# cliarie/radix-join

Hardware: AMD Instinct MI355X
Metric: probe_tuples_per_sec (higher is better)
Workload: dtype int32

## Files before the change

radix-join_amd/csrc/rj_context.hip:

```cpp
#include <dlfcn.h>

#include <algorithm>
#include <chrono>
#include <cstdlib>

#include "rj_internal.hpp"

namespace rj {

[[noreturn]] void launch_failed(const char* kernel, const char* what, bool unsupported) {
    throw_fmt(unsupported ? RJ_ERR_UNSUPPORTED : RJ_ERR_DEVICE, "launch %s: %s", kernel, what);
}

static int env_int(const char* name, int def) {
    const char* v = getenv(name);
    return v && *v ? atoi(v) : def;
}

void Tuning::from_env() {
    blocked_mid = env_int("RJ_TUNE_BLOCKED_MID", blocked_mid);
    mall_chunk = env_int("RJ_TUNE_MALL_CHUNK", mall_chunk);
    radix_bits = env_int("RJ_TUNE_RADIX_BITS", radix_bits);
    p1_bits = env_int("RJ_TUNE_P1_BITS", p1_bits);
    fine = env_int("RJ_TUNE_FINE", fine);
    pack = env_int("RJ_TUNE_PACK", pack);
    aos3 = env_int("RJ_TUNE_AOS3", aos3);
    aos_mid = env_int("RJ_TUNE_AOS_MID", aos_mid);
    tpg1 = env_int("RJ_TUNE_TPG1", tpg1);
    xcd_split = env_int("RJ_TUNE_XCD_SPLIT", xcd_split);
    tpg2 = env_int("RJ_TUNE_TPG2", tpg2);
    packed_side = env_int("RJ_TUNE_PACKED_SIDE", packed_side);
    xcd_min_rows = env_int("RJ_TUNE_XCD_MIN_ROWS", xcd_min_rows);
    spec_p1 = env_int("RJ_TUNE_SPEC_P1", spec_p1);
    spec_min_rows = env_int("RJ_TUNE_SPEC_MIN_ROWS", spec_min_rows);
    spec_sample = std::min(5, std::max(1, env_int("RJ_TUNE_SPEC_SAMPLE", spec_sample)));
    spec_z = std::max(0, env_int("RJ_TUNE_SPEC_Z", spec_z));
    spec_p2 = env_int("RJ_TUNE_SPEC_P2", spec_p2);
    spec2_min_rows = env_int("RJ_TUNE_SPEC2_MIN_ROWS", spec2_min_rows);
    spec2_sample = std::min(4, std::max(1, env_int("RJ_TUNE_SPEC2_SAMPLE", spec2_sample)));
    spec2_z = std::max(0, env_int("RJ_TUNE_SPEC2_Z", spec2_z));
    bcast = env_int("RJ_TUNE_BCAST", bcast);
    diag = env_int("RJ_DIAG", diag);
    varchar_dev_rows = env_int("RJ_TUNE_VARCHAR_DEV", varchar_dev_rows);
    vkey_hash_bits = env_int("RJ_DEBUG_VKEY_HASH_BITS", vkey_hash_bits);
    sync_upload = env_int("RJ_SYNC_UPLOAD", sync_upload);
    wide_carry = env_int("RJ_TUNE_WIDE_CARRY", wide_carry);
    fold_owner = env_int("RJ_TUNE_FOLD_OWNER", fold_owner);
    group_grid = env_int("RJ_TUNE_GROUP_GRID", group_grid);
    win_grid = env_int("RJ_TUNE_WIN_GRID", win_grid);
    map_grid = env_int("RJ_TUNE_MAP_GRID", map_grid);
    setop_grid = env_int("RJ_TUNE_SETOP_GRID", setop_grid);
    exchange_timeout_ms = env_int("RJ_EXCHANGE_TIMEOUT_MS", exchange_timeout_ms);
    bringup_timeout_ms = env_int("RJ_BRINGUP_TIMEOUT_MS", bringup_timeout_ms);
    debug_shard_fail = env_int("RJ_DEBUG_SHARD_FAIL", debug_shard_fail);
    debug_shard_fail_rank = env_int("RJ_DEBUG_SHARD_FAIL_RANK", debug_shard_fail_rank);
    if (const char* v = getenv("RJ_DEBUG_POISON"))
        debug_poison = (int)strtol(v, nullptr, 0) & 0x1ff;
}

static size_t round_size(size_t n) {
    const size_t small = 256, big = size_t(2) << 20;
    if (n < (size_t(1) << 20)) return (n + small - 1) / small * small;
    return (n + big - 1) / big * big;
}

void* DevPool::alloc(size_t bytes) {
    size_t need = round_size(bytes ? bytes : 1);
    int    best = -1;
    for (size_t i = 0; i < blocks_.size(); ++i) {
        Block& b = blocks_[i];
        if (!b.free || b.size < need) continue;
        if (b.size > need + need / 2 + (size_t(4) << 20)) continue;
        if (best < 0 || b.size < blocks_[best].size) best = (int)i;
    }
    if (best >= 0) {
        if (poison_) {
            hipError_t e = fill(blocks_[best].p, blocks_[best].size);
            if (e != hipSuccess) throw_fmt(RJ_ERR_DEVICE, "RJ_DEBUG_POISON: fill on alloc failed: %s", hipGetErrorString(e));
        }
        blocks_[best].free = false;
        in_use_ += blocks_[best].size;
        cached_ -= blocks_[best].size;
        return blocks_[best].p;
    }
    void*      p = nullptr;
    auto       t0 = std::chrono::steady_clock::now();
    hipError_t e = hipMalloc(&p, need);
    if (e != hipSuccess) {
        (void)hipGetLastError();
// ... 265 lines not shown
```

radix-join_amd/csrc/rj_internal.hpp:

```cpp
#pragma once
#include <hip/hip_runtime.h>

#include <atomic>
#include <cstdarg>
#include <cstdio>
#include <cstring>
#include <functional>
#include <map>
#include <memory>
#include <mutex>
#include <stdexcept>
#include <string>
#include <vector>

#include "../../include/rj.h"
#include "rj_comm.hpp"
#include "rj_device.hpp"
#include "rj_kernels.hpp"

namespace rj {

struct Context;

struct Error : std::runtime_error {
// ... 111 lines not shown
    uint64_t       page_rows_total = 0;
    BufP           page_rows;
    std::vector<uint32_t> page_rows_host;
    std::vector<uint8_t>        host_pages;
    std::vector<const uint8_t*> vc_pages;
    mutable BufP vc_dev, vc_dev_dir;
    bool                        skipped = false;
};

struct Table {
    Context*                 ctx = nullptr;
    uint64_t                 num_rows = 0;
    std::vector<TableColumn> cols;
};

struct ResultColumn {
    int32_t              type = 0;
    uint64_t             n_pages = 0;
    BufP                 dev_pages;
    std::vector<uint8_t> host_pages;
    struct Part {
        Context* ctx;
        BufP     pages;
        uint64_t n_pages;
    };
    std::vector<Part> more;
    uint64_t          n_first = 0;
};

struct Result {
    Context*                  ctx = nullptr;
    uint64_t                  num_rows = 0;
    std::vector<ResultColumn> cols;
};

struct Tuning {
    int blocked_mid = 1;
    int mall_chunk = 0;
    int radix_bits = 0;
    int p1_bits = 0;
    int fine = 1;
    int pack = 1;
    int aos3 = 1;
    int aos_mid = 2;
    int tpg1 = 0;
    int packed_side = 0;
    int tpg2 = 0;
    int xcd_min_rows = 40 << 20;
    int xcd_split = 1;
    int spec_p1 = 1;
    int spec_min_rows = 40 << 20;
    int spec_sample = 5;
    int spec_z = 60;
    int spec_p2 = 1;
    int spec2_min_rows = 40 << 20;
    int spec2_sample = 2;
    int spec2_z = 70;
    int bcast = 1;
    int diag = 0;
    int varchar_dev_rows = 200000;
    int vkey_hash_bits = 0;
    int sync_upload = 0;
    int wide_carry = 1;
    int fold_owner = 1;
    int group_grid = 0;
    int map_grid = 0;
    int win_grid = 0;
    int setop_grid = 0;
    int exchange_timeout_ms = 120000;
    int bringup_timeout_ms = 0;
    int debug_shard_fail = 0, debug_shard_fail_rank = 0;
    int debug_poison = 0;
    void from_env();
};

struct Context {
    Tuning      tune;
    int         device = 0;
    hipStream_t stream = nullptr;
    bool        own_stream = false;
    int         radix_bits_override = 0;
    DevPool     pool;
    Profiler    prof;
    LaunchLog   klog;
    std::string last_error;
    void*  pinned = nullptr;
    size_t pinned_bytes = 0;
    static constexpr size_t SMALL_PINNED = 32768;
    void*  pinned_small = nullptr;
    void*  small_pinned();
    hipStream_t copy_stream = nullptr;
    void*       pinned_up = nullptr;
    size_t      pinned_up_bytes = 0;
    hipStream_t upload_stream();
    hipStream_t aux = nullptr;
    hipStream_t aux_stream();
    void*       upload_staging(size_t bytes);
    Launch launch() {
        Launch L;
        L.stream = stream;
        L.self = this;
        L.timed = prof.on ? [](void* s, const char* n, hipEvent_t* a, hipEvent_t* b) {
            return static_cast<Context*>(s)->prof.timed(n, a, b);
        } : (bool (*)(void*, const char*, hipEvent_t*, hipEvent_t*)) nullptr;
        L.logged = klog.on ? [](void* s, const void* k) { static_cast<Context*>(s)->klog.add(k); }
                           : (void (*)(void*, const void*)) nullptr;
// ... 95 lines not shown
```

radix-join_amd/csrc/rj_kernels.hpp:

```cpp
#pragma once
#include <hip/hip_runtime.h>

#include "rj_device.hpp"

namespace rj {

struct Launch {
    hipStream_t stream;
    bool (*timed)(void* self, const char* name, hipEvent_t* start, hipEvent_t* stop);
    void* self;
    void (*logged)(void* self, const void* kernel);
};

[[noreturn]] void launch_failed(const char* kernel, const char* what, bool unsupported);

void launch_page_headers(const Launch& L, const uint8_t* pages, uint32_t n_pages, uint32_t rows_full,
                         uint32_t* page_rows, unsigned long long* flags);
void launch_rows_beyond(const Launch& L, const uint8_t* pages, uint32_t n_pages,
                        const uint32_t* row_base, uint64_t num_rows, unsigned long long* flag);
void launch_decode_pages(const Launch& L, const uint8_t* pages, uint32_t n_pages, int width,
                         const uint32_t* row_base, uint64_t num_rows, uint8_t* values,
                         uint8_t* valid);

void launch_gather(const Launch& L, const ColRef& src, const uint32_t* idx, uint64_t n,
                   const OutStream& dst, uint8_t* dst_valid);
void launch_outer_gather(const Launch& L, const ColRef& src, const uint32_t* idx, uint64_t n, uint8_t* dst,
                         uint8_t* dst_valid);
void launch_finish_pages(const Launch& L, uint8_t* pages, uint64_t n_rows, int width);
void launch_finish_streams(const Launch& L, uint8_t* const* pages, const int* widths, uint32_t n,
                           const unsigned long long* n_rows_dev, uint64_t cap_rows);
void launch_encode_nullable(const Launch& L, const uint8_t* values, const uint8_t* valid,
                            uint64_t n_rows, int width, uint8_t* pages);
void launch_pack_validity(const Launch& L, const uint8_t* v0, const uint8_t* v1, const uint8_t* v2, uint32_t n,
                          uint32_t* out);
void launch_split_records(const Launch& L, const SplitParams& sp, uint64_t n);
void launch_debug_stall(const Launch& L, uint32_t ms);

void launch_scan_bins(const Launch& L, const uint32_t* in, uint32_t n, uint32_t* off,
                      uint32_t* cursor);
void launch_scan_segments(const Launch& L, const uint32_t* hist, const uint32_t* seg_off,
                          uint32_t nseg, uint32_t F, uint32_t xcd_log2, uint32_t* off, uint32_t* cursor);
void launch_group_table(const Launch& L, const uint32_t* seg_off, uint32_t nseg,
                        uint32_t group_tuples, uint32_t* grp_start, const uint32_t* seg_end = nullptr);

void launch_pass_hist_src(const Launch& L, const TupleSrc& src, int key_words, const PassParams& pp,
                          uint32_t n_groups);
void launch_fine_hist_src(const Launch& L, const TupleSrc& src, int key_words, uint32_t shift,
                          uint32_t b1, uint32_t b2, uint32_t grid, uint32_t* fine, uint32_t xcd_tpg = 0,
                          uint32_t* coarse_x = nullptr);
void launch_fine_hist_words(const Launch& L, const Words& in, bool packed, uint32_t n, uint32_t shift,
                            uint32_t b1, uint32_t b2, uint32_t grid, uint32_t* fine, uint32_t xcd_tpg = 0,
                            uint32_t* coarse_x = nullptr);
void launch_scan_fine(const Launch& L, const uint32_t* fine, uint32_t F1, uint32_t F2,
                      uint32_t* off2, uint32_t* cursor2, uint32_t* off1, uint32_t* cursor1,
                      const uint32_t* coarse_x = nullptr);
void launch_pass_scatter_src(const Launch& L, const TupleSrc& src, int key_words, int carry_words,
                             const PassParams& pp, uint32_t n_groups, const Words& out, bool aos3 = false,
                             const SpecParams* spec = nullptr);
void launch_pass_sample_src(const Launch& L, const TupleSrc& src, int key_words, const PassParams& pp,
                            const SpecParams& sp, uint32_t n_groups);
void launch_spec_caps(const Launch& L, const uint32_t* sample, uint32_t nbins, uint32_t sample_log2, float z,
                      uint32_t cap_max, uint32_t* start, uint32_t* limit, unsigned long long* cursor);
void launch_spec_close(const Launch& L, const unsigned long long* cursor, const uint32_t* start, const uint32_t* limit,
                       uint32_t F, uint32_t* seg_end, uint32_t* oseg_off);
void launch_pass_hist_dense(const Launch& L, const Words& in, const PassParams& pp,
                            uint32_t n_groups);
void launch_pass_scatter_dense(const Launch& L, const Words& in, int n_words, int pair_word,
                               const PassParams& pp, uint32_t n_groups, const Words& out, bool aos3 = false);

void launch_pass_hist_digits(const Launch& L, const uint16_t* digits, const PassParams& pp, uint32_t n_groups);
void launch_pass_hist_aos3(const Launch& L, const uint32_t* in_tuples, const PassParams& pp, uint32_t n_groups);
void launch_pass_scatter_aos3(const Launch& L, const uint32_t* in_tuples, const PassParams& pp, uint32_t n_groups,
                              uint32_t* out_tuples);

void launch_pass_hist_packed(const Launch& L, const uint32_t* in_pairs, const PassParams& pp,
                             uint32_t n_groups);
void launch_pass_scatter_src_packed(const Launch& L, const TupleSrc& src, const PassParams& pp,
                                    uint32_t n_groups, uint32_t* out_pairs, bool blocked_out = false,
                                    const SpecParams* spec = nullptr);
void launch_pass_hist_blocked(const Launch& L, const uint32_t* in_blocked, const PassParams& pp, uint32_t n_groups);
void launch_pass_scatter_blocked(const Launch& L, const uint32_t* in_blocked, const PassParams& pp, uint32_t n_groups,
                                 uint32_t* out_pairs, bool blocked_out);
void launch_pass_scatter_packed(const Launch& L, const uint32_t* in_pairs, const PassParams& pp,
                                uint32_t n_groups, uint32_t* out_pairs);

void launch_heavy_tasks(const Launch& L, const uint32_t* offR, const uint32_t* offS, uint32_t NP,
                        uint32_t* tasks, uint32_t* n_heavy, uint32_t max_tasks, uint32_t off_pairs = 0);

void launch_last_sample(const Launch& L, const uint32_t* in_keys, bool blocked, const PassParams& pp, const LastParams& sp,
                        uint32_t n_groups);
void launch_last_caps(const Launch& L, const uint32_t* sample, uint32_t nseg, uint32_t F, uint32_t sample_log2, float z,
                      uint32_t cap_max, unsigned long long* seg_sum, uint32_t* pairs, uint32_t* limit,
                      uint32_t* cursor);
void launch_last_scatter_dense(const Launch& L, const Words& in, const PassParams& pp, uint32_t n_groups, const Words& out,
                               const LastParams& sp);
void launch_last_scatter_blocked(const Launch& L, const uint32_t* in_blocked, const PassParams& pp, uint32_t n_groups,
                                 uint32_t* out_pairs, const LastParams& sp);
void launch_last_close(const Launch& L, const uint32_t* cursor, const uint32_t* limit, uint32_t nbins,
                       uint32_t* pairs);

uint32_t join_partitions_per_workgroup(int key_words, int cw_build, const JoinParams& jp);
void launch_join(const Launch& L, int key_words, int cw_build, int cw_probe, const JoinParams& jp,
                 uint32_t grid);

void launch_join_bcast(const Launch& L, int key_words, int cw_build, int cw_probe,
                       const BcastParams& bp, uint32_t grid);

void launch_filter_bcast(const Launch& L, int key_words, int cw_preserved, const FilterParams& fp, uint32_t grid);
void launch_filter_join(const Launch& L, int key_words, int cw_preserved, const FilterParams& fp, uint32_t grid);
void launch_filter_nullkeys(const Launch& L, int key_words, int cw_preserved, const FilterParams& fp, uint32_t grid);

void launch_outer_bcast(const Launch& L, int key_words, int cw_optional, int cw_preserved, const OuterParams& op,
                        uint32_t grid);
// ... 105 lines not shown
```

radix-join_amd/csrc/rj_pages.hip:

```cpp
#include <hip/hip_ext.h>

#include "rj_kernels.hpp"
#include "rj_kernel_util.hpp"
#include "rj_tuple_util.hpp"

#include <algorithm>
#include <type_traits>

namespace rj {

__global__ __launch_bounds__(256) void k_page_headers(const uint8_t* pages, uint32_t n_pages,
                                                      uint32_t rows_full, uint32_t* page_rows,
                                                      unsigned long long* flags) {
    __shared__ unsigned long long s_irr[4], s_rows[4];
    const uint32_t     lane = threadIdx.x & 63u, wid = threadIdx.x >> 6;
    unsigned long long irr = 0, rows = 0;
    for (uint32_t p = blockIdx.x * 4u + wid; p < n_pages; p += gridDim.x * 4u) {
        const uint8_t* page = pages + (size_t)p * PAGE_BYTES;
        const uint32_t nr = *reinterpret_cast<const uint16_t*>(page);
        const uint32_t nb = (nr + 7) / 8;
        const uint8_t* bm = page + PAGE_BYTES - nb;
        bool           ones = true;
        const uint32_t boff = PAGE_BYTES - nb;
        if ((nr & 31u) == 0 && (boff & 3u) == 0) {
// ... 93 lines not shown
}

template <int WIDTH>
__global__ __launch_bounds__(256) void k_gather(ColRef src, const uint32_t* idx, uint64_t n,
                                                OutStream dst, uint8_t* dst_valid) {
    uint64_t i = (uint64_t)blockIdx.x * blockDim.x + threadIdx.x;
    if (i >= n) return;
    uint32_t r = idx ? idx[i] : (uint32_t)i;
    if (WIDTH == 4) {
        stream_store(dst, i, col_load32(src, r), 0u);
    } else {
        uint64_t v = col_load64(src, r);
        stream_store(dst, i, (uint32_t)v, (uint32_t)(v >> 32));
    }
    if (dst_valid) dst_valid[i] = src.valid ? src.valid[r] : (uint8_t)1;
}

template <int WIDTH>
__global__ __launch_bounds__(256) void k_outer_gather(ColRef src, const uint32_t* idx, uint64_t n, uint8_t* dst,
                                                      uint8_t* dst_valid) {
    const uint64_t i = (uint64_t)blockIdx.x * blockDim.x + threadIdx.x;
    if (i >= n) return;
    const uint32_t r = idx[i];
    const bool     there = r != OUTER_NO_ROW;
    if (WIDTH == 4)
        reinterpret_cast<uint32_t*>(dst)[i] = there ? col_load32(src, r) : 0u;
    else
        reinterpret_cast<uint64_t*>(dst)[i] = there ? col_load64(src, r) : 0ull;
    dst_valid[i] = there ? (src.valid ? src.valid[r] : (uint8_t)1) : (uint8_t)0;
}

__global__ __launch_bounds__(256) void k_finish_pages(uint8_t* pages, uint64_t n_rows,
                                                      uint32_t rows_full) {
    uint8_t*       page = pages + (size_t)blockIdx.x * PAGE_BYTES;
    const uint64_t first = (uint64_t)blockIdx.x * rows_full;
    const uint32_t nr = (uint32_t)min((uint64_t)rows_full, n_rows - first);
    const uint32_t nb = (nr + 7) / 8;
    if (threadIdx.x == 0) {
        reinterpret_cast<uint16_t*>(page)[0] = (uint16_t)nr;
        reinterpret_cast<uint16_t*>(page)[1] = (uint16_t)nr;
    }
    uint8_t* bm = page + PAGE_BYTES - nb;
    for (uint32_t k = threadIdx.x; k < nb; k += blockDim.x) {
        uint32_t bits = nr - k * 8u;
        bm[k] = bits >= 8 ? 0xff : (uint8_t)((1u << bits) - 1u);
    }
}

struct FinishStreams {
    uint8_t* pages[3];
    uint32_t rows_full[3];
    uint32_t n;
};
__global__ __launch_bounds__(256) void k_finish_streams(FinishStreams fs,
                                                        const unsigned long long* n_rows_dev,
                                                        uint64_t cap_rows) {
    const uint64_t n_rows = *n_rows_dev;
    if (n_rows > cap_rows) return;
    const uint32_t b = blockIdx.y, lane = threadIdx.x & 63u;
    const uint32_t rf = fs.rows_full[b];
    const uint64_t pg = (uint64_t)blockIdx.x * (blockDim.x >> 6) + (threadIdx.x >> 6);
    const uint64_t first = pg * rf;
    if (first >= n_rows) return;
    uint8_t*       page = fs.pages[b] + (size_t)pg * PAGE_BYTES;
    const uint32_t nr = (uint32_t)min((uint64_t)rf, n_rows - first);
    const uint32_t nb = (nr + 7) / 8;
    if (lane == 0) *reinterpret_cast<uint32_t*>(page) = nr | (nr << 16);
    uint8_t* bm = page + PAGE_BYTES - nb;
    if (nr == rf && (nr & 31u) == 0 && ((PAGE_BYTES - nb) & 3u) == 0) {
        for (uint32_t k = lane; k < nb / 4; k += 64) reinterpret_cast<uint32_t*>(bm)[k] = 0xffffffffu;
        return;
    }
    if (nr == rf && rf == ROWS64) {
        static_assert(ROWS64 == 1007 && ((PAGE_BYTES - 126 + 2) & 3u) == 0, "bitmap layout of a full 8-byte page");
        if (lane == 0) *reinterpret_cast<uint16_t*>(bm) = 0xffffu;
        if (lane < 31) reinterpret_cast<uint32_t*>(bm + 2)[lane] = lane == 30 ? 0x7fffffffu : 0xffffffffu;
        return;
    }
    for (uint32_t k = lane; k < nb; k += 64) {
        uint32_t bits = nr - k * 8u;
        bm[k] = bits >= 8 ? 0xff : (uint8_t)((1u << bits) - 1u);
    }
}

template <int WIDTH>
__global__ __launch_bounds__(256) void k_encode_nullable(const uint8_t* values, const uint8_t* valid,
                                                         uint64_t n_rows, uint8_t* pages) {
    __shared__ uint32_t s_w[4];
    constexpr uint32_t  RF = WIDTH == 4 ? ROWS32 : ROWS64;
    uint8_t*            page = pages + (size_t)blockIdx.x * PAGE_BYTES;
    const uint64_t      first = (uint64_t)blockIdx.x * RF;
    const uint32_t      nr = (uint32_t)min((uint64_t)RF, n_rows - first);
    const uint32_t      nb = (nr + 7) / 8;
    uint8_t*            out_vals = page + (WIDTH == 4 ? HDR32 : HDR64);
    uint8_t*            bm = page + PAGE_BYTES - nb;
    const uint32_t      lane = threadIdx.x & 63u, wid = threadIdx.x >> 6;
    uint32_t            running = 0;
    for (uint32_t base = 0; base < nr; base += 256) {
        uint32_t i = base + threadIdx.x;
        bool     bit = i < nr ? valid[first + i] != 0 : false;
        uint64_t mask = __ballot(bit);
        uint32_t pre = lane_prefix(mask);
        if (lane == 0) s_w[wid] = (uint32_t)__popcll(mask);
        __syncthreads();
        uint32_t wpre = 0, tot = 0;
#pragma unroll
        for (uint32_t k = 0; k < 4; ++k) {
            uint32_t c = s_w[k];
            if (k < wid) wpre += c;
            tot += c;
        }
        if (bit) {
            uint32_t vi = running + wpre + pre;
            if (WIDTH == 4)
                reinterpret_cast<uint32_t*>(out_vals)[vi] =
                    reinterpret_cast<const uint32_t*>(values)[first + i];
            else
                reinterpret_cast<uint64_t*>(out_vals)[vi] =
                    reinterpret_cast<const uint64_t*>(values)[first + i];
        }
        if (lane < 8) {
            uint32_t byte_idx = (base >> 3) + wid * 8u + lane;
            if (byte_idx < nb) bm[byte_idx] = (uint8_t)(mask >> (lane * 8u));
        }
        running += tot;
        __syncthreads();
    }
    if (threadIdx.x == 0) {
        reinterpret_cast<uint16_t*>(page)[0] = (uint16_t)nr;
        reinterpret_cast<uint16_t*>(page)[1] = (uint16_t)running;
    }
}

__global__ __launch_bounds__(256) void k_pack_validity(const uint8_t* v0, const uint8_t* v1, const uint8_t* v2,
// ... 42 lines not shown
               num_rows, flag);
}

void launch_decode_pages(const Launch& L, const uint8_t* pages, uint32_t n_pages, int width,
                         const uint32_t* row_base, uint64_t num_rows, uint8_t* values,
                         uint8_t* valid) {
    if (!n_pages) return;
    if (width == 4)
        RJ_KLAUNCH(L, "decode_pages", (k_decode_pages<4>), n_pages, 256, pages, row_base, num_rows,
                   values, valid);
    else
        RJ_KLAUNCH(L, "decode_pages", (k_decode_pages<8>), n_pages, 256, pages, row_base, num_rows,
                   values, valid);
}

void launch_gather(const Launch& L, const ColRef& src, const uint32_t* idx, uint64_t n,
                   const OutStream& dst, uint8_t* dst_valid) {
    if (!n) return;
    uint32_t grid = (uint32_t)((n + 255) / 256);
    if (src.width == 4)
        RJ_KLAUNCH(L, "gather", (k_gather<4>), grid, 256, src, idx, n, dst, dst_valid);
    else
        RJ_KLAUNCH(L, "gather", (k_gather<8>), grid, 256, src, idx, n, dst, dst_valid);
}

void launch_outer_gather(const Launch& L, const ColRef& src, const uint32_t* idx, uint64_t n, uint8_t* dst,
                         uint8_t* dst_valid) {
    if (!n) return;
    const uint32_t grid = (uint32_t)((n + 255) / 256);
    if (src.width == 4)
        RJ_KLAUNCH(L, "outer_gather", (k_outer_gather<4>), grid, 256, src, idx, n, dst, dst_valid);
    else
        RJ_KLAUNCH(L, "outer_gather", (k_outer_gather<8>), grid, 256, src, idx, n, dst, dst_valid);
}

void launch_finish_pages(const Launch& L, uint8_t* pages, uint64_t n_rows, int width) {
    if (!n_rows) return;
    uint32_t rf = width == 4 ? ROWS32 : ROWS64;
    uint32_t np = (uint32_t)((n_rows + rf - 1) / rf);
    RJ_KLAUNCH(L, "finish_pages", k_finish_pages, np, 256, pages, n_rows, rf);
}

void launch_finish_streams(const Launch& L, uint8_t* const* pages, const int* widths, uint32_t n,
                           const unsigned long long* n_rows_dev, uint64_t cap_rows) {
    if (!n || !cap_rows) return;
    FinishStreams fs{};
    fs.n = n;
    uint64_t max_pages = 0;
    for (uint32_t i = 0; i < n && i < 3; ++i) {
        fs.pages[i] = pages[i];
        fs.rows_full[i] = widths[i] == 4 ? ROWS32 : ROWS64;
        max_pages = std::max<uint64_t>(max_pages, (cap_rows + fs.rows_full[i] - 1) / fs.rows_full[i]);
    }
    RJ_KLAUNCH(L, "finish_pages", k_finish_streams, dim3((uint32_t)((max_pages + 3) / 4), n), 256, fs,
               n_rows_dev, cap_rows);
}

void launch_encode_nullable(const Launch& L, const uint8_t* values, const uint8_t* valid,
                            uint64_t n_rows, int width, uint8_t* pages) {
    if (!n_rows) return;
    uint32_t rf = width == 4 ? ROWS32 : ROWS64;
    uint32_t np = (uint32_t)((n_rows + rf - 1) / rf);
    if (width == 4)
        RJ_KLAUNCH(L, "encode_nullable", (k_encode_nullable<4>), np, 256, values, valid, n_rows,
                   pages);
    else
        RJ_KLAUNCH(L, "encode_nullable", (k_encode_nullable<8>), np, 256, values, valid, n_rows,
                   pages);
}

void launch_pack_validity(const Launch& L, const uint8_t* v0, const uint8_t* v1, const uint8_t* v2, uint32_t n,
                          uint32_t* out) {
    if (!n) return;
    RJ_KLAUNCH(L, "pack_validity", k_pack_validity, (n + 255) / 256, 256, v0, v1, v2, n, out);
}

void launch_split_records(const Launch& L, const SplitParams& sp, uint64_t n) {
    if (!n) return;
    RJ_KLAUNCH(L, "split_records", k_split_records, (uint32_t)((n + 255) / 256), 256, sp, n);
}

void launch_debug_stall(const Launch& L, uint32_t ms) {
    int dev = 0, khz = 0;
    (void)hipGetDevice(&dev);
    if (hipDeviceGetAttribute(&khz, hipDeviceAttributeWallClockRate, dev) != hipSuccess || khz <= 0) khz = 100000;
    RJ_KLAUNCH(L, "debug_stall", k_debug_stall, 1, 64, (unsigned long long)ms * (unsigned long long)khz);
}

void prewarm_pages(const Launch& L, uint32_t* zeroed) {
    const uint8_t* const v = reinterpret_cast<const uint8_t*>(zeroed);
    RJ_KLAUNCH(L, "prewarm", k_pack_validity, 1, 256, v, v, v, 0u, zeroed);
}

}
```

radix-join_amd/csrc/rj_partition.hip:

```cpp
#include <hip/hip_ext.h>

#include "rj_kernels.hpp"
#include "rj_kernel_util.hpp"
#include "rj_tuple_util.hpp"

#include <algorithm>
#include <type_traits>

namespace rj {

template <int MODE>
__global__ __launch_bounds__(1024) void k_scan_bins(const uint32_t* in, const uint32_t* in_end, uint32_t n,
                                                    uint32_t div, uint32_t* off, uint32_t* cursor) {
    __shared__ uint32_t s_wsum[16];
    const uint32_t      chunk = (n + 1023u) / 1024u;
    const uint32_t      b = threadIdx.x * chunk;
    const uint32_t      e = min(n, b + chunk);
    uint32_t            sum = 0;
    for (uint32_t i = b; i < e; ++i) {
        uint32_t v = MODE == 0 ? in[i] : ((in_end ? in_end[i] : in[i + 1]) - in[i] + div - 1u) / div;
        sum += v;
    }
    uint32_t total;
    uint32_t run = block_excl_scan(sum, s_wsum, total);
// ... 590 lines not shown
    while (hi - lo > 1) {
        uint32_t mid = (lo + hi) >> 1;
        if (pp.grp_start[mid] - pp.grp_base <= g)
            lo = mid;
        else
            hi = mid;
    }
    seg = lo >> pp.oseg_shift;
    uint32_t gi = g - (pp.grp_start[lo] - pp.grp_base);
    uint64_t b = (uint64_t)pp.seg_off[lo] + (uint64_t)gi * gt;
    begin = (uint32_t)b;
    end = (uint32_t)min((uint64_t)(pp.seg_end ? pp.seg_end[lo] : pp.seg_off[lo + 1]), b + gt);
    return begin < end;
}

template <class L, class = void>
struct loader_needs_begin : std::false_type {};
template <class L>
struct loader_needs_begin<L, std::enable_if_t<L::kNeedsBegin>> : std::true_type {};

template <class Loader>
__global__ __launch_bounds__(PT_THREADS) void k_pass_hist(Loader ld, PassParams pp) {
    __shared__ uint32_t s_h[PT_MAXF];
    uint32_t            seg, begin, end;
    if (!group_range(pp, blockIdx.x, seg, begin, end)) return;
    const uint32_t F = 1u << pp.fanout_log2, mask = F - 1u;
    for (uint32_t d = threadIdx.x; d < F; d += PT_THREADS) s_h[d] = 0;
    lds_barrier();
    for (uint32_t base = begin; base < end; base += PT_TILE) {
        uint32_t hk[PT_ITEMS];
        uint32_t ok;
        if constexpr (loader_needs_begin<Loader>::value)
            ok = ld.key_tile(base, begin, end, hk);
        else
            ok = ld.key_tile(base, end, hk);
#pragma unroll
        for (int j = 0; j < PT_ITEMS; ++j) {
            if ((ok >> j) & 1u) atomicAdd(&s_h[pass_digit(pp, hk[j], mask)], 1u);
        }
    }
    if constexpr (loader_needs_begin<Loader>::value) {
        uint32_t hx;
        if (ld.extra(begin, end, hx)) atomicAdd(&s_h[pass_digit(pp, hx, mask)], 1u);
    }
    lds_barrier();
    for (uint32_t d = threadIdx.x; d < F; d += PT_THREADS) {
        uint32_t c = s_h[d];
        if (c) atomicAdd(&pp.hist[(((size_t)seg * F + d) << pp.xcd_log2) | (blockIdx.x & ((1u << pp.xcd_log2) - 1u))], c);
    }
}

static_assert((PT_TILE & (PT_TILE - 1)) == 0, "a tile's sample slice is a power-of-two fraction of it");
template <int KW>
__global__ __launch_bounds__(PT_THREADS) void k_pass_sample(TupleSrc s, PassParams pp, SpecParams sp) {
    __shared__ uint32_t s_h[PT_MAXF];
    uint32_t            seg, begin, end;
    if (!group_range(pp, blockIdx.x, seg, begin, end)) return;
    const uint32_t F = 1u << pp.fanout_log2, mask = F - 1u;
    for (uint32_t d = threadIdx.x; d < F; d += PT_THREADS) s_h[d] = 0;
    lds_barrier();
    const uint32_t slog = (uint32_t)__builtin_ctz((unsigned)PT_TILE) - sp.sample_log2, slice = 1u << slog;
    const uint32_t ntiles = (end - begin + (uint32_t)PT_TILE - 1u) / (uint32_t)PT_TILE;
    const uint32_t total = ntiles << slog;
    constexpr int  U = 4;
    for (uint32_t i0 = threadIdx.x; i0 < total; i0 += U * PT_THREADS) {
        uint32_t lo[U], hi[U];
        bool     ok[U];
#pragma unroll
        for (int u = 0; u < U; ++u) {
            const uint32_t i = i0 + u * PT_THREADS, ic = min(i, total - 1u);
            const uint32_t t = ic >> slog, r = ic & (slice - 1u);
            const uint32_t tb = begin + t * (uint32_t)PT_TILE, rows = min((uint32_t)PT_TILE, end - tb);
            const uint32_t rot = ((tb / (uint32_t)PT_TILE) * 7u << slog) & ((uint32_t)PT_TILE - 1u);
            const uint32_t at = rows > slice ? min(rot, rows - slice) : 0u;
            const uint32_t row = tb + min(at + r, rows - 1u);
            ok[u] = i < total && r < rows;
            if constexpr (KW == 1) {
                lo[u] = col_load32(s.key, row);
                hi[u] = 0;
            } else {
                const uint64_t k = col_load64(s.key, row);
                lo[u] = (uint32_t)k;
                hi[u] = (uint32_t)(k >> 32);
            }
            if (s.key.valid && !s.key.valid[row]) ok[u] = false;
        }
#pragma unroll
        for (int u = 0; u < U; ++u) {
            uint32_t h;
            if constexpr (KW == 1) {
                h = s.prehashed ? lo[u] : fmix32(lo[u]);
            } else {
                const uint64_t k = (uint64_t)lo[u] | ((uint64_t)hi[u] << 32);
                if (s.key_f64 && (k & 0x7ff0000000000000ull) == 0x7ff0000000000000ull && (k & 0x000fffffffffffffull))
                    ok[u] = false;
                h = (uint32_t)fmix64(k);
            }
            if (ok[u]) atomicAdd(&s_h[pass_digit(pp, h, mask)], 1u);
        }
    }
    lds_barrier();
    for (uint32_t d = threadIdx.x; d < F; d += PT_THREADS) {
        uint32_t c = s_h[d];
        if (c) atomicAdd(&pp.hist[(((size_t)seg * F + d) << pp.xcd_log2) | (blockIdx.x & ((1u << pp.xcd_log2) - 1u))], c);
    }
}

__global__ __launch_bounds__(1024) void k_spec_caps(const uint32_t* sample, uint32_t nbins, uint32_t sample_log2, float z,
                                                    uint32_t cap_max, uint32_t* start, uint32_t* limit,
                                                    unsigned long long* cursor) {
    __shared__ unsigned long long s_sum[1024];
    const uint32_t                chunk = (nbins + 1023u) / 1024u;
    const uint32_t                b = min(nbins, threadIdx.x * chunk), e = min(nbins, b + chunk);
    auto                          cap_of = [&](uint32_t c) -> unsigned long long {
        const double zz = (double)z, x = (double)c + zz * sqrt((double)c + 1.0) + 0.5 * zz * zz;
        const unsigned long long t = (unsigned long long)ceil(ldexp(x, (int)sample_log2));
        return (t + 31ull) & ~31ull;
    };
    unsigned long long sum = 0;
    for (uint32_t i = b; i < e; ++i) sum += cap_of(sample[i]);
    s_sum[threadIdx.x] = sum;
    __syncthreads();
    unsigned long long run = 0;
    for (uint32_t k = 0; k < threadIdx.x; ++k) run += s_sum[k];
    for (uint32_t i = b; i < e; ++i) {
        const unsigned long long nx = run + cap_of(sample[i]);
        const uint32_t           st = (uint32_t)min(run, (unsigned long long)cap_max);
        const uint32_t           lim = (uint32_t)min(nx, (unsigned long long)cap_max);
        start[i] = st;
        limit[i] = lim;
        cursor[i] = (unsigned long long)st | ((unsigned long long)(lim - st) << 32);
        run = nx;
    }
}

__global__ __launch_bounds__(PT_MAXF) void k_spec_close(const unsigned long long* cursor, const uint32_t* start,
                                                        const uint32_t* limit, uint32_t F, uint32_t* seg_end,
                                                        uint32_t* oseg_off) {
    __shared__ uint32_t s_wsum[PT_MAXF / 64];
    const uint32_t      d = threadIdx.x;
    uint32_t            v = 0;
    if (d < F)
        for (uint32_t x = 0; x < 8; ++x) {
            const uint32_t i = (d << 3) | x, en = min((uint32_t)cursor[i], limit[i]);
            seg_end[i] = en;
            v += en - start[i];
        }
    uint32_t       total;
    const uint32_t ex = block_excl_scan(v, s_wsum, total);
    if (d < F) oseg_off[d] = ex;
    if (d == 0) oseg_off[F] = total;
// ... 265 lines not shown
    const uint32_t i = blockIdx.x * 256u + threadIdx.x;
    if (i < nbins) pairs[2 * (size_t)i + 1] = min(cursor[i], limit[i]);
}

__global__ void k_heavy_tasks(const uint32_t* offR, const uint32_t* offS, uint32_t NP,
                              uint32_t* tasks, uint32_t* n_heavy, uint32_t max_tasks, uint32_t off_pairs) {
    uint32_t q = blockIdx.x * blockDim.x + threadIdx.x;
    if (q >= NP) return;
    const uint32_t ir = q << (off_pairs & 1u), is = q << (off_pairs >> 1);
    uint32_t sb = offS[is], se = offS[is + 1];
    uint32_t len = se - sb;
    if (len <= JN_HEAVY || offR[ir + 1] == offR[ir]) return;
    uint32_t nt = (len + JN_HEAVY - 1) / JN_HEAVY;
    uint32_t b = atomicAdd(n_heavy, nt);
    for (uint32_t t = 0; t < nt; ++t) {
        uint32_t k = b + t;
        if (k >= max_tasks) break;
        tasks[3 * k + 0] = q;
        tasks[3 * k + 1] = (uint32_t)((uint64_t)sb + (uint64_t)t * JN_HEAVY);
        tasks[3 * k + 2] = (uint32_t)min((uint64_t)se, (uint64_t)sb + (uint64_t)(t + 1) * JN_HEAVY);
    }
}

void launch_scan_bins(const Launch& L, const uint32_t* in, uint32_t n, uint32_t* off,
                      uint32_t* cursor) {
    RJ_KLAUNCH(L, "scan_bins", (k_scan_bins<0>), 1, 1024, in, (const uint32_t*)nullptr, n, 1u, off, cursor);
}

void launch_scan_segments(const Launch& L, const uint32_t* hist, const uint32_t* seg_off,
                          uint32_t nseg, uint32_t F, uint32_t xcd_log2, uint32_t* off, uint32_t* cursor) {
    RJ_KLAUNCH(L, "scan_segments", k_scan_segments, nseg, PT_MAXF, hist, seg_off, nseg, F, xcd_log2, off,
               cursor);
}

void launch_group_table(const Launch& L, const uint32_t* seg_off, uint32_t nseg,
                        uint32_t group_tuples, uint32_t* grp_start, const uint32_t* seg_end) {
    RJ_KLAUNCH(L, "group_table", (k_scan_bins<1>), 1, 1024, seg_off, seg_end, nseg, group_tuples, grp_start,
               (uint32_t*)nullptr);
}

void launch_pass_hist_src(const Launch& L, const TupleSrc& src, int key_words, const PassParams& pp,
                          uint32_t n_groups) {
    if (!n_groups) return;
    if (key_words == 1) {
        SrcLoader<1, 0> ld{src};
        RJ_KLAUNCH(L, "pass1_hist", (k_pass_hist<SrcLoader<1, 0>>), n_groups, PT_THREADS, ld, pp);
    } else {
        SrcLoader<2, 0> ld{src};
        RJ_KLAUNCH(L, "pass1_hist", (k_pass_hist<SrcLoader<2, 0>>), n_groups, PT_THREADS, ld, pp);
    }
}

void launch_pass_sample_src(const Launch& L, const TupleSrc& src, int key_words, const PassParams& pp,
                            const SpecParams& sp, uint32_t n_groups) {
    if (!n_groups) return;
    if (key_words == 1)
        RJ_KLAUNCH(L, "pass1_sample", (k_pass_sample<1>), n_groups, PT_THREADS, src, pp, sp);
    else
        RJ_KLAUNCH(L, "pass1_sample", (k_pass_sample<2>), n_groups, PT_THREADS, src, pp, sp);
}

void launch_spec_caps(const Launch& L, const uint32_t* sample, uint32_t nbins, uint32_t sample_log2, float z,
                      uint32_t cap_max, uint32_t* start, uint32_t* limit, unsigned long long* cursor) {
    RJ_KLAUNCH(L, "spec_caps", k_spec_caps, 1, 1024, sample, nbins, sample_log2, z, cap_max, start, limit, cursor);
}

void launch_spec_close(const Launch& L, const unsigned long long* cursor, const uint32_t* start, const uint32_t* limit,
                       uint32_t F, uint32_t* seg_end, uint32_t* oseg_off) {
    RJ_KLAUNCH(L, "spec_close", k_spec_close, 1, PT_MAXF, cursor, start, limit, F, seg_end, oseg_off);
}

void launch_fine_hist_src(const Launch& L, const TupleSrc& src, int key_words, uint32_t shift,
                          uint32_t b1, uint32_t b2, uint32_t grid, uint32_t* fine, uint32_t xcd_tpg,
                          uint32_t* coarse_x) {
    if (!grid || !src.n_rows) return;
    if (key_words == 1) {
        SrcLoader<1, 0> ld{src};
        RJ_KLAUNCH(L, "pass1_hist", (k_fine_hist<SrcLoader<1, 0>>), grid, PT_THREADS, ld, src.n_rows,
                   shift, b1, b2, fine, xcd_tpg, coarse_x);
    } else {
        SrcLoader<2, 0> ld{src};
        RJ_KLAUNCH(L, "pass1_hist", (k_fine_hist<SrcLoader<2, 0>>), grid, PT_THREADS, ld, src.n_rows,
                   shift, b1, b2, fine, xcd_tpg, coarse_x);
    }
}

void launch_fine_hist_words(const Launch& L, const Words& in, bool packed, uint32_t n, uint32_t shift,
                            uint32_t b1, uint32_t b2, uint32_t grid, uint32_t* fine, uint32_t xcd_tpg,
                            uint32_t* coarse_x) {
    if (!grid || !n) return;
    if (packed) {
        PackedLoader ld{reinterpret_cast<const uint2*>(in.w[0])};
        RJ_KLAUNCH(L, "pass1_hist", (k_fine_hist<PackedLoader>), grid, PT_THREADS, ld, n, shift, b1, b2, fine,
                   xcd_tpg, coarse_x);
    } else {
        DenseLoader ld{in};
        RJ_KLAUNCH(L, "pass1_hist", (k_fine_hist<DenseLoader>), grid, PT_THREADS, ld, n, shift, b1, b2, fine,
                   xcd_tpg, coarse_x);
    }
}

void launch_scan_fine(const Launch& L, const uint32_t* fine, uint32_t F1, uint32_t F2,
                      uint32_t* off2, uint32_t* cursor2, uint32_t* off1, uint32_t* cursor1,
                      const uint32_t* coarse_x) {
    RJ_KLAUNCH(L, "scan_fine", k_scan_fine, F1, PT_MAXF, fine, F1, F2, off2, cursor2, off1, cursor1,
               coarse_x);
}

template <int KW, int CW, int WIDE = WIDE_NONE>
static void scatter_src_t(const Launch& L, const TupleSrc& src, const PassParams& pp,
                          uint32_t n_groups, const Words& out, const SpecParams* spec) {
    SrcLoader<KW, CW, WIDE> ld{src};
// ... 208 lines not shown
```

radix-join_amd/csrc/rj_radix.hip:

```cpp
#include "rj_radix.hpp"

#include <algorithm>

#include "rj_radix_plan.hpp"

namespace rj {

void read_back(Context* ctx, void* dst, const void* src, size_t bytes) {
    try {
        RJ_HIP(hipMemcpyAsync(dst, src, bytes, hipMemcpyDeviceToHost, ctx->stream));
        ctx->sync();
    } catch (...) {
        (void)hipStreamSynchronize(ctx->stream);
        throw;
    }
}

namespace {

RadixFacts facts_of(const PartitionRequest& rq) {
    RadixFacts f;
    f.n = rq.ws ? rq.ws->n : (rq.src ? rq.src->n_rows : 0);
    f.KW = rq.KW, f.CW = rq.CW, f.bits = rq.bits, f.shift0 = rq.shift0, f.single_pass = rq.single_pass;
    f.word_src = rq.ws != nullptr, f.word_src_packed = rq.ws && rq.ws->packed;
// ... 195 lines not shown
        if (fine_xcd) {
            coarse_x = ctx->buf((uint64_t)F1 * 8 * 4);
            RJ_HIP(hipMemsetAsync(coarse_x->p, 0, (uint64_t)F1 * 8 * 4, ctx->stream));
        }
        uint32_t* cx = fine_xcd ? coarse_x->as<uint32_t>() : nullptr;
        if (rq.ws)
            launch_fine_hist_words(L, rq.ws->w, rq.ws->packed, (uint32_t)n, rq.shift0, pl.pbits[0], pl.pbits[1], pl.fine_grid,
                                   fh->as<uint32_t>(), fine_xcd ? pl.tpg_first : 0u, cx);
        else
            launch_fine_hist_src(L, src, rq.KW, rq.shift0, pl.pbits[0], pl.pbits[1], pl.fine_grid, fh->as<uint32_t>(),
                                 fine_xcd ? pl.tpg_first : 0u, cx);
        launch_scan_fine(L, fh->as<uint32_t>(), F1, F2, fine_off->as<uint32_t>(), fine_cursor->as<uint32_t>(),
                         coarse_off->as<uint32_t>(), coarse_cursor->as<uint32_t>(), cx);
    }

    void exact_bins(PassRun& r) {
        const uint64_t bins = r.ps.bins;
        r.hist = ctx->buf((bins << r.pp.xcd_log2) * 4);
        r.off = ctx->buf((bins + 1) * 4);
        r.cursor = ctx->buf((bins << r.pp.xcd_log2) * 4);
        RJ_HIP(hipMemsetAsync(r.hist->p, 0, (bins << r.pp.xcd_log2) * 4, ctx->stream));
        r.pp.hist = r.hist->as<uint32_t>();
        r.pp.cursor = r.cursor->as<uint32_t>();
    }

    void exact_histogram(PassRun& r) {
        const uint32_t G = r.ps.n_groups, prev = (r.p + 1) % 2;
        switch (r.ps.hist) {
        case RadixHist::Src: launch_pass_hist_src(L, src, rq.KW, r.pp, G); break;
        case RadixHist::Digits: launch_pass_hist_digits(L, SIDE[prev]->as<uint16_t>(), r.pp, G); break;
        case RadixHist::Aos3: launch_pass_hist_aos3(L, MID[prev]->as<uint32_t>(), r.pp, G); break;
        case RadixHist::Blocked: launch_pass_hist_blocked(L, cur.w[0], r.pp, G); break;
        case RadixHist::Packed: launch_pass_hist_packed(L, cur.w[0], r.pp, G); break;
        case RadixHist::Dense: launch_pass_hist_dense(L, cur, r.pp, G); break;
        default: throw_fmt(RJ_ERR_DEVICE, "radix plan: pass %u has no exact histogram", r.p);
        }
    }

    void sample_first(PassRun& r) {
        const uint32_t spec_s = (uint32_t)ctx->tune.spec_sample;
        const uint32_t nb = (uint32_t)r.ps.bins << 3;
        r.hist = ctx->buf((uint64_t)nb * 4);
        r.off = ctx->buf((r.ps.bins + 1) * 4);
        r.cursor = ctx->buf((uint64_t)nb * 8);
        spec_start = ctx->buf((uint64_t)nb * 4);
        spec_limit = ctx->buf((uint64_t)nb * 4);
        spec_end = ctx->buf((uint64_t)nb * 4);
        RJ_HIP(hipMemsetAsync(r.hist->p, 0, (uint64_t)nb * 4, ctx->stream));
        r.pp.hist = r.hist->as<uint32_t>();
        r.sp.cursor = r.cursor->as<unsigned long long>();
        r.sp.flag = rq.spec_flag;
        r.sp.sink = (uint32_t)pl.spec_cap_max;
        r.sp.sample_log2 = spec_s;
        launch_pass_sample_src(L, src, rq.KW, r.pp, r.sp, r.ps.n_groups);
        launch_spec_caps(L, r.pp.hist, nb, spec_s, (float)(ctx->tune.spec_z / 10.0), (uint32_t)pl.spec_cap_max,
                         spec_start->as<uint32_t>(), spec_limit->as<uint32_t>(), r.sp.cursor);
    }

    void sample_last(PassRun& r) {
        const uint32_t spec2_s = (uint32_t)ctx->tune.spec2_sample;
        const uint32_t nb = (uint32_t)r.ps.bins, nseg_in = r.ps.nseg_in;
        r.hist = ctx->buf((uint64_t)nb * 4);
        r.off = ctx->buf((uint64_t)nb * 8);
        r.cursor = ctx->buf((uint64_t)nb * 4);
        last_limit = ctx->buf((uint64_t)nb * 4);
        last_seg_sum = ctx->buf((uint64_t)r.ps.n_oseg * 8);
        RJ_HIP(hipMemsetAsync(r.hist->p, 0, (uint64_t)nb * 4, ctx->stream));
        r.pp.hist = r.hist->as<uint32_t>();
        r.lp.cursor32 = r.cursor->as<uint32_t>();
        r.lp.limit = last_limit->as<uint32_t>();
        r.lp.flag = rq.spec_flag;
        r.lp.sink = (uint32_t)pl.spec2_cap_max;
        r.lp.sample_log2 = spec2_s;
        PassParams ps = r.pp;
        ps.tiles_per_group = LAST_SAMPLE_TPG;
        last_grp = ctx->buf(((uint64_t)nseg_in + 1) * 4);
        launch_group_table(L, r.pp.seg_off, nseg_in, LAST_SAMPLE_TPG * (uint32_t)PT_TILE, last_grp->as<uint32_t>(), r.in_end);
        ps.grp_start = last_grp->as<uint32_t>();
        launch_last_sample(L, cur.w[0], P.packed, ps, r.lp, r.ps.sample_groups);
        launch_last_caps(L, r.pp.hist, r.ps.n_oseg, r.F, spec2_s, (float)(ctx->tune.spec2_z / 10.0), (uint32_t)pl.spec2_cap_max,
                         last_seg_sum->as<unsigned long long>(), r.off->as<uint32_t>(), last_limit->as<uint32_t>(), r.lp.cursor32);
    }

    void send_sizes_to_host(PassRun& r) {
        const uint64_t bytes = (r.ps.bins + 1) * 4;
        if (bytes > Context::SMALL_PINNED / 4) throw_fmt(RJ_ERR_DEVICE, "chunked pass: too many segments");
        RJ_HIP(hipMemcpyAsync(ctx->small_pinned(), r.off->p, bytes, hipMemcpyDeviceToHost, ctx->stream));
        chunk_ev.make();
        RJ_HIP(hipEventRecord(chunk_ev.e, ctx->stream));
    }

    void chunked_pass(PassRun& r) {
        const PassParams& pp = r.pp;
        const uint32_t    nseg_in = r.ps.nseg_in, F = r.F;
        RJ_HIP(hipEventSynchronize(chunk_ev.e));
        const uint32_t* hoff = static_cast<const uint32_t*>(ctx->small_pinned());
        const uint64_t  gt = (uint64_t)pp.tiles_per_group * PT_TILE;
        std::vector<uint32_t> gstart(nseg_in + 1, 0);
        for (uint32_t sgi = 0; sgi < nseg_in; ++sgi)
            gstart[sgi + 1] = gstart[sgi] + (uint32_t)(((uint64_t)(hoff[sgi + 1] - hoff[sgi]) + gt - 1) / gt);
        Event e_in, e_aux;
        e_in.make();
        e_aux.make();
        hipStream_t aux = ctx->aux_stream();
        RJ_HIP(hipEventRecord(e_in.e, ctx->stream));
        RJ_HIP(hipStreamWaitEvent(aux, e_in.e, 0));
        Launch L2 = L;
// ... 76 lines not shown
```

Before: 35.07 billion.

## Make sample kernel persistent with software-pipelined loads; batch pages in finish kernel

The pass-1 sample kernel becomes a grid-stride persistent kernel capped at about twice the compute-unit count. Each block walks several groups and keeps two or three batches of loads in flight while it counts the earlier batch into the shared histogram. This is meant to hide load latency and cut per-block launch and histogram-init overhead. Separately, the finish-pages kernel now makes each wavefront handle eight pages and adds a fast path for full 4-byte-row pages. The sample kernel now rejects multi-segment inputs outright, and the histogram flush happens once per block instead of once per group.

```diff
diff --git a/radix-join_amd/csrc/rj_context.hip b/radix-join_amd/csrc/rj_context.hip
--- a/radix-join_amd/csrc/rj_context.hip
+++ b/radix-join_amd/csrc/rj_context.hip
@@ -35,6 +35,7 @@
     spec_min_rows = env_int("RJ_TUNE_SPEC_MIN_ROWS", spec_min_rows);
     spec_sample = std::min(5, std::max(1, env_int("RJ_TUNE_SPEC_SAMPLE", spec_sample)));
     spec_z = std::max(0, env_int("RJ_TUNE_SPEC_Z", spec_z));
+    sample_grid = std::max(0, env_int("RJ_TUNE_SAMPLE_GRID", sample_grid));
     spec_p2 = env_int("RJ_TUNE_SPEC_P2", spec_p2);
     spec2_min_rows = env_int("RJ_TUNE_SPEC2_MIN_ROWS", spec2_min_rows);
     spec2_sample = std::min(4, std::max(1, env_int("RJ_TUNE_SPEC2_SAMPLE", spec2_sample)));
diff --git a/radix-join_amd/csrc/rj_internal.hpp b/radix-join_amd/csrc/rj_internal.hpp
--- a/radix-join_amd/csrc/rj_internal.hpp
+++ b/radix-join_amd/csrc/rj_internal.hpp
@@ -187,6 +187,7 @@
     int spec_min_rows = 40 << 20;
     int spec_sample = 5;
     int spec_z = 60;
+    int sample_grid = 0;
     int spec_p2 = 1;
     int spec2_min_rows = 40 << 20;
     int spec2_sample = 2;
diff --git a/radix-join_amd/csrc/rj_kernels.hpp b/radix-join_amd/csrc/rj_kernels.hpp
--- a/radix-join_amd/csrc/rj_kernels.hpp
+++ b/radix-join_amd/csrc/rj_kernels.hpp
@@ -58,7 +58,7 @@
                              const PassParams& pp, uint32_t n_groups, const Words& out, bool aos3 = false,
                              const SpecParams* spec = nullptr);
 void launch_pass_sample_src(const Launch& L, const TupleSrc& src, int key_words, const PassParams& pp,
-                            const SpecParams& sp, uint32_t n_groups);
+                            const SpecParams& sp, uint32_t n_groups, uint32_t max_grid);
 void launch_spec_caps(const Launch& L, const uint32_t* sample, uint32_t nbins, uint32_t sample_log2, float z,
                       uint32_t cap_max, uint32_t* start, uint32_t* limit, unsigned long long* cursor);
 void launch_spec_close(const Launch& L, const unsigned long long* cursor, const uint32_t* start, const uint32_t* limit,
diff --git a/radix-join_amd/csrc/rj_pages.hip b/radix-join_amd/csrc/rj_pages.hip
--- a/radix-join_amd/csrc/rj_pages.hip
+++ b/radix-join_amd/csrc/rj_pages.hip
@@ -169,6 +169,7 @@
     uint32_t rows_full[3];
     uint32_t n;
 };
+constexpr uint32_t FINISH_PPW = 8;
 __global__ __launch_bounds__(256) void k_finish_streams(FinishStreams fs,
                                                         const unsigned long long* n_rows_dev,
                                                         uint64_t cap_rows) {
@@ -176,27 +177,29 @@
     if (n_rows > cap_rows) return;
     const uint32_t b = blockIdx.y, lane = threadIdx.x & 63u;
     const uint32_t rf = fs.rows_full[b];
-    const uint64_t pg = (uint64_t)blockIdx.x * (blockDim.x >> 6) + (threadIdx.x >> 6);
-    const uint64_t first = pg * rf;
-    if (first >= n_rows) return;
-    uint8_t*       page = fs.pages[b] + (size_t)pg * PAGE_BYTES;
-    const uint32_t nr = (uint32_t)min((uint64_t)rf, n_rows - first);
-    const uint32_t nb = (nr + 7) / 8;
-    if (lane == 0) *reinterpret_cast<uint32_t*>(page) = nr | (nr << 16);
-    uint8_t* bm = page + PAGE_BYTES - nb;
-    if (nr == rf && (nr & 31u) == 0 && ((PAGE_BYTES - nb) & 3u) == 0) {
-        for (uint32_t k = lane; k < nb / 4; k += 64) reinterpret_cast<uint32_t*>(bm)[k] = 0xffffffffu;
-        return;
-    }
-    if (nr == rf && rf == ROWS64) {
-        static_assert(ROWS64 == 1007 && ((PAGE_BYTES - 126 + 2) & 3u) == 0, "bitmap layout of a full 8-byte page");
-        if (lane == 0) *reinterpret_cast<uint16_t*>(bm) = 0xffffu;
-        if (lane < 31) reinterpret_cast<uint32_t*>(bm + 2)[lane] = lane == 30 ? 0x7fffffffu : 0xffffffffu;
-        return;
-    }
-    for (uint32_t k = lane; k < nb; k += 64) {
-        uint32_t bits = nr - k * 8u;
-        bm[k] = bits >= 8 ? 0xff : (uint8_t)((1u << bits) - 1u);
+    const uint64_t pg0 = ((uint64_t)blockIdx.x * (blockDim.x >> 6) + (threadIdx.x >> 6)) * FINISH_PPW;
+    for (uint32_t k = 0; k < FINISH_PPW; ++k) {
+        const uint64_t pg = pg0 + k, first = pg * rf;
+        if (first >= n_rows) return;
+        uint8_t*       page = fs.pages[b] + (size_t)pg * PAGE_BYTES;
+        const uint32_t nr = (uint32_t)min((uint64_t)rf, n_rows - first);
+        const uint32_t nb = (nr + 7) / 8;
+        if (lane == 63) *reinterpret_cast<uint32_t*>(page) = nr | (nr << 16);
+        uint8_t* bm = page + PAGE_BYTES - nb;
+        if (nr == rf && rf == ROWS32) {
+            static_assert(ROWS32 % 32 == 0 && ROWS32 / 32 < 64 && ((PAGE_BYTES - ROWS32 / 8) & 3u) == 0,
+                          "bitmap layout of a full 4-byte page");
+            if (lane < ROWS32 / 32) reinterpret_cast<uint32_t*>(bm)[lane] = 0xffffffffu;
+        } else if (nr == rf && rf == ROWS64) {
+            static_assert(ROWS64 == 1007 && ((PAGE_BYTES - 126 + 2) & 3u) == 0, "bitmap layout of a full 8-byte page");
+            if (lane == 62) *reinterpret_cast<uint16_t*>(bm) = 0xffffu;
+            if (lane < 31) reinterpret_cast<uint32_t*>(bm + 2)[lane] = lane == 30 ? 0x7fffffffu : 0xffffffffu;
+        } else {
+            for (uint32_t i = lane; i < nb; i += 64) {
+                uint32_t bits = nr - i * 8u;
+                bm[i] = bits >= 8 ? 0xff : (uint8_t)((1u << bits) - 1u);
+            }
+        }
     }
 }
 
@@ -345,7 +348,8 @@
         fs.rows_full[i] = widths[i] == 4 ? ROWS32 : ROWS64;
         max_pages = std::max<uint64_t>(max_pages, (cap_rows + fs.rows_full[i] - 1) / fs.rows_full[i]);
     }
-    RJ_KLAUNCH(L, "finish_pages", k_finish_streams, dim3((uint32_t)((max_pages + 3) / 4), n), 256, fs,
+    const uint64_t per_wg = 4 * FINISH_PPW;
+    RJ_KLAUNCH(L, "finish_pages", k_finish_streams, dim3((uint32_t)((max_pages + per_wg - 1) / per_wg), n), 256, fs,
                n_rows_dev, cap_rows);
 }
 
diff --git a/radix-join_amd/csrc/rj_partition.hip b/radix-join_amd/csrc/rj_partition.hip
--- a/radix-join_amd/csrc/rj_partition.hip
+++ b/radix-join_amd/csrc/rj_partition.hip
@@ -666,51 +666,94 @@
 
 static_assert((PT_TILE & (PT_TILE - 1)) == 0, "a tile's sample slice is a power-of-two fraction of it");
 template <int KW>
-__global__ __launch_bounds__(PT_THREADS) void k_pass_sample(TupleSrc s, PassParams pp, SpecParams sp) {
+__global__ __launch_bounds__(PT_THREADS, 8) void k_pass_sample(TupleSrc s, PassParams pp, SpecParams sp) {
     __shared__ uint32_t s_h[PT_MAXF];
-    uint32_t            seg, begin, end;
-    if (!group_range(pp, blockIdx.x, seg, begin, end)) return;
-    const uint32_t F = 1u << pp.fanout_log2, mask = F - 1u;
+    const uint32_t      F = 1u << pp.fanout_log2, mask = F - 1u;
     for (uint32_t d = threadIdx.x; d < F; d += PT_THREADS) s_h[d] = 0;
     lds_barrier();
     const uint32_t slog = (uint32_t)__builtin_ctz((unsigned)PT_TILE) - sp.sample_log2, slice = 1u << slog;
-    const uint32_t ntiles = (end - begin + (uint32_t)PT_TILE - 1u) / (uint32_t)PT_TILE;
-    const uint32_t total = ntiles << slog;
     constexpr int  U = 4;
-    for (uint32_t i0 = threadIdx.x; i0 < total; i0 += U * PT_THREADS) {
+    struct Step {
         uint32_t lo[U], hi[U];
+        uint8_t  valid[U];
         bool     ok[U];
+    };
+    uint32_t g = blockIdx.x, at0 = 0, seg = 0, begin = 0, end = 0, total = 0;
+    auto     open = [&](uint32_t grp) -> bool {
+        if (!group_range(pp, grp, seg, begin, end)) return false;
+        total = ((end - begin + (uint32_t)PT_TILE - 1u) / (uint32_t)PT_TILE) << slog;
+        return true;
+    };
+    auto issue = [&](Step& st) {
 #pragma unroll
         for (int u = 0; u < U; ++u) {
-            const uint32_t i = i0 + u * PT_THREADS, ic = min(i, total - 1u);
+            const uint32_t i = at0 + threadIdx.x + u * PT_THREADS, ic = min(i, total - 1u);
             const uint32_t t = ic >> slog, r = ic & (slice - 1u);
             const uint32_t tb = begin + t * (uint32_t)PT_TILE, rows = min((uint32_t)PT_TILE, end - tb);
             const uint32_t rot = ((tb / (uint32_t)PT_TILE) * 7u << slog) & ((uint32_t)PT_TILE - 1u);
             const uint32_t at = rows > slice ? min(rot, rows - slice) : 0u;
             const uint32_t row = tb + min(at + r, rows - 1u);
-            ok[u] = i < total && r < rows;
+            st.ok[u] = i < total && r < rows;
             if constexpr (KW == 1) {
-                lo[u] = col_load32(s.key, row);
-                hi[u] = 0;
+                st.lo[u] = col_load32(s.key, row);
+                st.hi[u] = 0;
             } else {
                 const uint64_t k = col_load64(s.key, row);
-                lo[u] = (uint32_t)k;
-                hi[u] = (uint32_t)(k >> 32);
-            }
-            if (s.key.valid && !s.key.valid[row]) ok[u] = false;
-        }
+                st.lo[u] = (uint32_t)k;
+                st.hi[u] = (uint32_t)(k >> 32);
+            }
+            st.valid[u] = s.key.valid ? s.key.valid[row] : (uint8_t)1;
+        }
+    };
+    auto count = [&](const Step& st) {
 #pragma unroll
         for (int u = 0; u < U; ++u) {
+            bool     ok = st.ok[u] && st.valid[u];
             uint32_t h;
             if constexpr (KW == 1) {
-                h = s.prehashed ? lo[u] : fmix32(lo[u]);
+                h = s.prehashed ? st.lo[u] : fmix32(st.lo[u]);
             } else {
-                const uint64_t k = (uint64_t)lo[u] | ((uint64_t)hi[u] << 32);
+                const uint64_t k = (uint64_t)st.lo[u] | ((uint64_t)st.hi[u] << 32);
                 if (s.key_f64 && (k & 0x7ff0000000000000ull) == 0x7ff0000000000000ull && (k & 0x000fffffffffffffull))
-                    ok[u] = false;
+                    ok = false;
                 h = (uint32_t)fmix64(k);
             }
-            if (ok[u]) atomicAdd(&s_h[pass_digit(pp, h, mask)], 1u);
+            if (ok) atomicAdd(&s_h[pass_digit(pp, h, mask)], 1u);
+        }
+    };
+    constexpr int D = KW == 1 ? 3 : 2;
+    Step          st[D] = {};
+    bool          full[D];
+    bool          more = open(g);
+    auto          next = [&] {
+        at0 += U * PT_THREADS;
+        if (at0 >= total) {
+            g += gridDim.x;
+            at0 = 0;
+            more = open(g);
+        }
+    };
+#pragma unroll
+    for (int d = 0; d < D; ++d) {
+        full[d] = more;
+        if (more) {
+            issue(st[d]);
+            next();
+        }
+    }
+    for (bool done = false; !done;) {
+#pragma unroll
+        for (int d = 0; d < D; ++d) {
+            if (!full[d]) {
+                done = true;
+                break;
+            }
+            count(st[d]);
+            full[d] = more;
+            if (more) {
+                issue(st[d]);
+                next();
+            }
         }
     }
     lds_barrier();
@@ -1082,12 +1125,14 @@
 }
 
 void launch_pass_sample_src(const Launch& L, const TupleSrc& src, int key_words, const PassParams& pp,
-                            const SpecParams& sp, uint32_t n_groups) {
-    if (!n_groups) return;
+                            const SpecParams& sp, uint32_t n_groups, uint32_t max_grid) {
+    if (!n_groups) return;
+    if (pp.seg_off) launch_failed("k_pass_sample", "samples one input segment only", true);
+    const uint32_t grid = std::min(n_groups, std::max(8u, max_grid & ~7u));
     if (key_words == 1)
-        RJ_KLAUNCH(L, "pass1_sample", (k_pass_sample<1>), n_groups, PT_THREADS, src, pp, sp);
+        RJ_KLAUNCH(L, "pass1_sample", (k_pass_sample<1>), grid, PT_THREADS, src, pp, sp);
     else
-        RJ_KLAUNCH(L, "pass1_sample", (k_pass_sample<2>), n_groups, PT_THREADS, src, pp, sp);
+        RJ_KLAUNCH(L, "pass1_sample", (k_pass_sample<2>), grid, PT_THREADS, src, pp, sp);
 }
 
 void launch_spec_caps(const Launch& L, const uint32_t* sample, uint32_t nbins, uint32_t sample_log2, float z,
diff --git a/radix-join_amd/csrc/rj_radix.hip b/radix-join_amd/csrc/rj_radix.hip
--- a/radix-join_amd/csrc/rj_radix.hip
+++ b/radix-join_amd/csrc/rj_radix.hip
@@ -271,7 +271,8 @@
         r.sp.flag = rq.spec_flag;
         r.sp.sink = (uint32_t)pl.spec_cap_max;
         r.sp.sample_log2 = spec_s;
-        launch_pass_sample_src(L, src, rq.KW, r.pp, r.sp, r.ps.n_groups);
+        const uint32_t sample_grid = ctx->tune.sample_grid > 0 ? (uint32_t)ctx->tune.sample_grid : (uint32_t)ctx->compute_units() * 2u;
+        launch_pass_sample_src(L, src, rq.KW, r.pp, r.sp, r.ps.n_groups, sample_grid);
         launch_spec_caps(L, r.pp.hist, nb, spec_s, (float)(ctx->tune.spec_z / 10.0), (uint32_t)pl.spec_cap_max,
                          spec_start->as<uint32_t>(), spec_limit->as<uint32_t>(), r.sp.cursor);
     }
```

Result: slower. 33.79 billion (-3.6%).
